# rongzhao-zhang/EfficientQ

Measured on AMD Instinct MI355X. Metric: ptq_calibration_throughput, higher is better.
Workload: dtype i8xi8->i32 (exact) for the Gram systems and per-iteration loss convs of the layers with quantised input, f32/f64 elsewhere

## Files before the change

### efficientq_amd/csrc/solve.hip

```cpp
#include <cstdlib>
#include <vector>
#include "common.h"

namespace effq {

typedef float f32x16 __attribute__((ext_vector_type(16)));
typedef double f64x4 __attribute__((ext_vector_type(4)));
typedef float f32x4 __attribute__((ext_vector_type(4)));

static inline int round_up(int v, int m) { return (v + m - 1) / m * m; }

constexpr int NBK = 64;
constexpr int LDA_S = 66;
constexpr int LDB_S = 80;

__global__ __launch_bounds__(256) void k_build_a64(const float* __restrict__ A0, int n, int npad, int has_bias,
                                                   double rho, double eta, double* __restrict__ A64) {
  const size_t tot = (size_t)npad * npad;
  const size_t stride = (size_t)gridDim.x * blockDim.x;
  for (size_t e = (size_t)blockIdx.x * blockDim.x + threadIdx.x; e < tot; e += stride) {
    const int i = (int)(e / npad), j = (int)(e % npad);
    double v = 0.0;
    if (i < n && j < n) {
      v = (double)A0[(size_t)i * n + j];
// ... 516 lines not shown
  constexpr int CPW = NBK / 16;
  auto invert64 = [&](int off) {
    double reg[CPW];
#pragma unroll
    for (int j = 0; j < CPW; ++j) reg[j] = M[(off + lane) * PF_LD + off + wid * CPW + j];
    gj_invert_regs<CPW>(reg, fcol, lane, wid);
#pragma unroll
    for (int j = 0; j < CPW; ++j) M[(off + lane) * PF_LD + off + wid * CPW + j] = reg[j];
    lds_barrier();
  };
  auto zero = []() {
    f64x4 z;
#pragma unroll
    for (int r = 0; r < 4; ++r) z[r] = 0.0;
    return z;
  };
  auto tile_store = [&](int rb, int cb, f64x4 v, double sgn) {
#pragma unroll
    for (int r = 0; r < 4; ++r) M[(rb + tr * 16 + lk + 4 * r) * PF_LD + cb + tc * 16 + lr] = sgn * v[r];
  };
  auto tile_load = [&](int rb, int cb) {
    f64x4 v;
#pragma unroll
    for (int r = 0; r < 4; ++r) v[r] = M[(rb + tr * 16 + lk + 4 * r) * PF_LD + cb + tc * 16 + lr];
    return v;
  };
  invert64(0);
  if (mk == 2) {
    f64x4 z = mm16(zero(), M + (NBK + tr * 16) * PF_LD, PF_LD, 1, M + tc * 16, PF_LD, 1, NBK, lr, lk);
    lds_barrier();
    tile_store(NBK, 0, z, 1.0);
    lds_barrier();
    f64x4 sacc = tile_load(NBK, NBK);
#pragma unroll
    for (int r = 0; r < 4; ++r) sacc[r] = -sacc[r];
    sacc = mm16(sacc, M + (NBK + tr * 16) * PF_LD, PF_LD, 1, M + NBK + tc * 16, PF_LD, 1, NBK, lr, lk);
    tile_store(NBK, NBK, sacc, -1.0);
    lds_barrier();
    invert64(NBK);
    f64x4 w = mm16(zero(), M + (NBK + tr * 16) * PF_LD + NBK, PF_LD, 1, M + NBK * PF_LD + tc * 16, PF_LD, 1, NBK, lr, lk);
    tile_store(0, NBK, w, 1.0);
    lds_barrier();
    f64x4 d = tile_load(0, 0);
    d = mm16(d, M + NBK * PF_LD + tr * 16, 1, PF_LD, M + NBK + tc * 16, PF_LD, 1, NBK, lr, lk);
    tile_store(0, 0, d, 1.0);
    lds_barrier();
  }
  const int nd = mk * NBK;
  for (int e = tid; e < nd * nd; e += 1024) {
    const int i = e / nd, j = e % nd;
    double v;
    if (i < NBK && j >= NBK)
      v = -M[(j - NBK) * PF_LD + NBK + i];
    else if (i >= NBK && j < NBK)
      v = -M[(i - NBK) * PF_LD + NBK + j];
    else
      v = M[i * PF_LD + j];
    Dw[e] = v;
  }
}

__global__ __launch_bounds__(256) void k_mirror_blocks(double* __restrict__ D, int nd) {
  const size_t tot = (size_t)nd * nd;
  for (size_t e = (size_t)blockIdx.x * blockDim.x + threadIdx.x; e < tot; e += (size_t)gridDim.x * blockDim.x) {
    const int i = (int)(e / nd), j = (int)(e % nd);
    if ((i / NBK) > (j / NBK)) D[e] = D[(size_t)j * nd + i];
  }
}

__global__ __launch_bounds__(256) void k_build_b(const float* __restrict__ B0, const float* __restrict__ W0,
                                                 const float* __restrict__ b0, const float* __restrict__ G,
                                                 const float* __restrict__ dual, int c2, int n, int has_bias,
                                                 float rho, float eta, float* __restrict__ Bm, int ldb, int c2p,
                                                 const float* __restrict__ wprev, float shift) {
  const size_t tot = (size_t)c2p * ldb;
  const size_t stride = (size_t)gridDim.x * blockDim.x;
  const int nw = n - has_bias;
  for (size_t e = (size_t)blockIdx.x * blockDim.x + threadIdx.x; e < tot; e += stride) {
    const int r = (int)(e / ldb), k = (int)(e % ldb);
    float v = 0.0f;
    if (r < c2 && k < n) {
      if (k < nw) {
        const size_t wi = (size_t)r * nw + k;
        v = B0[(size_t)r * n + k] + eta * W0[wi];
        v = v + rho * (G[wi] - dual[wi]);
        if (wprev != nullptr) v = v + shift * wprev[wi];
      } else {
        v = B0[(size_t)r * n + k] + eta * b0[r];
      }
    }
    Bm[e] = v;
  }
}

__global__ __launch_bounds__(256) void k_build_b4(const float* __restrict__ B0, const float* __restrict__ W0,
                                                  const float* __restrict__ b0, const float* __restrict__ G,
                                                  const float* __restrict__ dual, int c2, int n, int has_bias,
                                                  float rho, float eta, float* __restrict__ Bm, int ldb,
                                                  const float* __restrict__ wprev, float shift) {
  __builtin_amdgcn_s_setprio(2);

  const int r = blockIdx.y;
  const int nw = n - has_bias;
  float* out = Bm + (size_t)r * ldb;
  for (int k = (blockIdx.x * blockDim.x + threadIdx.x) * 4; k < ldb; k += gridDim.x * blockDim.x * 4) {
    float4 v = make_float4(0.f, 0.f, 0.f, 0.f);
    if (r < c2 && k < nw) {
      const size_t wi = (size_t)r * nw + k;
      const float* bp = B0 + (size_t)r * n + k;
      const float4 w0 = *reinterpret_cast<const float4*>(W0 + wi), g = *reinterpret_cast<const float4*>(G + wi),
                   du = *reinterpret_cast<const float4*>(dual + wi);
      v.x = bp[0] + eta * w0.x;
      v.y = bp[1] + eta * w0.y;
      v.z = bp[2] + eta * w0.z;
      v.w = bp[3] + eta * w0.w;
      v.x = v.x + rho * (g.x - du.x);
      v.y = v.y + rho * (g.y - du.y);
      v.z = v.z + rho * (g.z - du.z);
      v.w = v.w + rho * (g.w - du.w);
      if (wprev != nullptr) {
        const float4 wp = *reinterpret_cast<const float4*>(wprev + wi);
        v.x = v.x + shift * wp.x;
        v.y = v.y + shift * wp.y;
        v.z = v.z + shift * wp.z;
        v.w = v.w + shift * wp.w;
      }
    } else if (r < c2 && k == nw && has_bias) {
      v.x = B0[(size_t)r * n + k] + eta * b0[r];
    }
    *reinterpret_cast<float4*>(out + k) = v;
  }
}

__global__ __launch_bounds__(256) void k_prox_reduce4(const float* __restrict__ part, int ldp, int nsplit, int c2, int n,
                                                      int has_bias, float* __restrict__ wstar, float* __restrict__ bstar) {
  __builtin_amdgcn_s_setprio(2);

  const int r = blockIdx.y;
  const int nw = n - has_bias;
  const size_t tot = (size_t)c2 * ldp;
  const float* row = part + (size_t)r * ldp;
  for (int k = (blockIdx.x * blockDim.x + threadIdx.x) * 4; k < ldp; k += gridDim.x * blockDim.x * 4) {
    if (k >= n) continue;
    float4 v = *reinterpret_cast<const float4*>(row + k);
    for (int z = 1; z < nsplit; ++z) {
      const float4 t = *reinterpret_cast<const float4*>(row + (size_t)z * tot + k);
      v.x += t.x;
      v.y += t.y;
      v.z += t.z;
      v.w += t.w;
    }
    if (k < nw)
      *reinterpret_cast<float4*>(wstar + (size_t)r * nw + k) = v;
    else
      bstar[r] = v.x;
  }
}

constexpr int PBK = 32, PLD = PBK + 4;

template <int MT, int WM, int WN, int NTN>
__global__ __launch_bounds__(256) void k_prox_gemm(const float* __restrict__ Bm, int ldb, const float* __restrict__ Ainv,
                                                   int lda, int n, int c2, int has_bias, float* __restrict__ wstar,
                                                   float* __restrict__ bstar, float* __restrict__ part, int ldp) {
  __builtin_amdgcn_s_setprio(2);

  constexpr int BM = 32 * MT * WM, BN = 32 * WN * NTN;
  constexpr int NA = BM * 8 / 256, NB = BN * 8 / 256;
  static_assert(WM * WN == 4 && NA >= 1 && NB >= 1, "4 waves");
  __shared__ __attribute__((aligned(16))) float As[BM * PLD];
  __shared__ __attribute__((aligned(16))) float Bs[BN * PLD];
  const int tid = threadIdx.x, lane = tid & 63, wid = tid >> 6;
  const int li = lane & 31, lh = lane >> 5;
  const int wm = wid / WN, wn = wid % WN;
  const int row0 = blockIdx.y * BM, col0 = blockIdx.x * BN;

  f32x16 acc[MT][NTN];
#pragma unroll
  for (int m = 0; m < MT; ++m)
#pragma unroll
    for (int t = 0; t < NTN; ++t)
#pragma unroll
      for (int r = 0; r < 16; ++r) acc[m][t][r] = 0.0f;

  f32x4 ra[NA], rb[NB];
  const float* pa[NA];
  const float* pb[NB];
#pragma unroll
  for (int q = 0; q < NA; ++q) {
    const int u = tid + q * 256, r = u >> 3, c4 = u & 7;
    pa[q] = Bm + (size_t)(row0 + r) * ldb + c4 * 4;
  }
#pragma unroll
  for (int q = 0; q < NB; ++q) {
    const int u = tid + q * 256, r = u >> 3, c4 = u & 7;
    pb[q] = Ainv + (size_t)min(col0 + r, n - 1) * lda + c4 * 4;
  }
#define EFFQ_PROX_FETCH(k0)                                                         \
  {                                                                                 \
    _Pragma("unroll") for (int q = 0; q < NA; ++q)                                  \
        ra[q] = *reinterpret_cast<const f32x4*>(pa[q] + (k0));                      \
    _Pragma("unroll") for (int q = 0; q < NB; ++q)                                  \
        rb[q] = *reinterpret_cast<const f32x4*>(pb[q] + (k0));                      \
  }
  const int nkt = ldb / PBK;
  const int kt0 = (int)(((long long)nkt * blockIdx.z) / gridDim.z);
  const int nk = (int)(((long long)nkt * (blockIdx.z + 1)) / gridDim.z);
  EFFQ_PROX_FETCH(kt0 * PBK)
  for (int kt = kt0; kt < nk; ++kt) {
    lds_barrier();
#pragma unroll
    for (int q = 0; q < NA; ++q) {
      const int u = tid + q * 256;
      *reinterpret_cast<f32x4*>(&As[(u >> 3) * PLD + (u & 7) * 4]) = ra[q];
    }
#pragma unroll
    for (int q = 0; q < NB; ++q) {
      const int u = tid + q * 256;
      *reinterpret_cast<f32x4*>(&Bs[(u >> 3) * PLD + (u & 7) * 4]) = rb[q];
    }
    lds_barrier();
    EFFQ_PROX_FETCH(min(kt + 1, nk - 1) * PBK)
    __builtin_amdgcn_sched_barrier(0);
#pragma unroll
    for (int q = 0; q < 4; ++q) {
      f32x4 a[MT], b[NTN];
#pragma unroll
      for (int m = 0; m < MT; ++m)
        a[m] = *reinterpret_cast<const f32x4*>(&As[((wm * MT + m) * 32 + li) * PLD + q * 8 + 4 * lh]);
#pragma unroll
      for (int t = 0; t < NTN; ++t)
        b[t] = *reinterpret_cast<const f32x4*>(&Bs[((wn * NTN + t) * 32 + li) * PLD + q * 8 + 4 * lh]);
#pragma unroll
      for (int m = 0; m < MT; ++m)
#pragma unroll
        for (int t = 0; t < NTN; ++t)
#pragma unroll
          for (int e = 0; e < 4; ++e)
            acc[m][t] = __builtin_amdgcn_mfma_f32_32x32x2f32(a[m][e], b[t][e], acc[m][t], 0, 0, 0);
    }
  }
#undef EFFQ_PROX_FETCH
  const int nw = n - has_bias;
  if (gridDim.z > 1) {
    float* P = part + (size_t)blockIdx.z * c2 * ldp;
#pragma unroll
    for (int m = 0; m < MT; ++m)
#pragma unroll
      for (int t = 0; t < NTN; ++t) {
        const int col = col0 + (wn * NTN + t) * 32 + li;
#pragma unroll
        for (int r = 0; r < 16; ++r) {
          const int row = row0 + (wm * MT + m) * 32 + (r & 3) + 8 * (r >> 2) + 4 * lh;
          if (row < c2 && col < n) P[(size_t)row * ldp + col] = acc[m][t][r];
        }
      }
    return;
  }
#pragma unroll
  for (int m = 0; m < MT; ++m)
#pragma unroll
    for (int t = 0; t < NTN; ++t) {
      const int col = col0 + (wn * NTN + t) * 32 + li;
#pragma unroll
      for (int r = 0; r < 16; ++r) {
        const int row = row0 + (wm * MT + m) * 32 + (r & 3) + 8 * (r >> 2) + 4 * lh;
        if (row < c2 && col < n) {
          if (col < nw)
            wstar[(size_t)row * nw + col] = acc[m][t][r];
          else
            bstar[row] = acc[m][t][r];
        }
      }
    }
}


typedef __bf16 bf16x8 __attribute__((ext_vector_type(8)));
typedef __bf16 bf16x4 __attribute__((ext_vector_type(4)));
constexpr int B3_K = 16;
constexpr int B3_LD = B3_K + 8;

__device__ __forceinline__ void split3(const f32x4 v, bf16x4& p0, bf16x4& p1, bf16x4& p2) {
#pragma unroll
  for (int e = 0; e < 4; ++e) {
    const __bf16 b0 = (__bf16)v[e];
    const float r1 = v[e] - (float)b0;
    const __bf16 b1 = (__bf16)r1;
    const float r2 = r1 - (float)b1;
    p0[e] = b0;
    p1[e] = b1;
    p2[e] = (__bf16)r2;
  }
}

template <int BM, int BN, int WM, int WN>
__global__ __launch_bounds__(512) void k_prox_gemm_b3(const float* __restrict__ Bm, int ldb, const float* __restrict__ Ainv,
                                                      int lda, int n, int c2, int has_bias, float* __restrict__ wstar,
                                                      float* __restrict__ bstar, float* __restrict__ part, int ldp) {
  __builtin_amdgcn_s_setprio(2);
  constexpr int MT = BM / WM / 32, NT = BN / WN / 32;
  constexpr int NA = BM * 4 / 512, NB = BN * 4 / 512;
  constexpr int STAGE = 3 * (BM + BN) * B3_LD;
  static_assert(WM * WN == 8 && MT >= 1 && NT >= 1 && NA >= 1 && NB >= 1, "8 waves");
  extern __shared__ __attribute__((aligned(16))) unsigned char b3_lds[];
  __bf16* lds = reinterpret_cast<__bf16*>(b3_lds);
  const int tid = threadIdx.x, lane = tid & 63, wid = tid >> 6;
  const int li = lane & 31, lh = lane >> 5;
  const int wm = wid / WN, wn = wid % WN;
  const int row0 = blockIdx.y * BM, col0 = blockIdx.x * BN;

  f32x16 acc[MT][NT];
#pragma unroll
  for (int m = 0; m < MT; ++m)
#pragma unroll
    for (int t = 0; t < NT; ++t)
#pragma unroll
      for (int r = 0; r < 16; ++r) acc[m][t][r] = 0.0f;

  f32x4 ra[NA], rb[NB];
  const float* pa[NA];
  const float* pb[NB];
#pragma unroll
  for (int q = 0; q < NA; ++q) {
    const int u = tid + q * 512, r = u >> 2, c4 = u & 3;
    pa[q] = Bm + (size_t)(row0 + r) * ldb + c4 * 4;
  }
#pragma unroll
  for (int q = 0; q < NB; ++q) {
    const int u = tid + q * 512, r = u >> 2, c4 = u & 3;
    pb[q] = Ainv + (size_t)min(col0 + r, n - 1) * lda + c4 * 4;
  }
#define EFFQ_B3_FETCH(k0)                                                           \
  {                                                                                 \
    _Pragma("unroll") for (int q = 0; q < NA; ++q)                                  \
        ra[q] = *reinterpret_cast<const f32x4*>(pa[q] + (k0));                      \
    _Pragma("unroll") for (int q = 0; q < NB; ++q)                                  \
        rb[q] = *reinterpret_cast<const f32x4*>(pb[q] + (k0));                      \
  }
#define EFFQ_B3_STORE(stage)                                                                        \
  {                                                                                                 \
    __bf16* As_ = lds + (stage) * STAGE;                                                            \
    __bf16* Bs_ = As_ + 3 * BM * B3_LD;                                                             \
    _Pragma("unroll") for (int q = 0; q < NA; ++q) {                                                \
      const int u = tid + q * 512, off = (u >> 2) * B3_LD + (u & 3) * 4;                            \
      bf16x4 p0, p1, p2;                                                                            \
      split3(ra[q], p0, p1, p2);                                                                    \
      *reinterpret_cast<bf16x4*>(&As_[off]) = p0;                                                   \
      *reinterpret_cast<bf16x4*>(&As_[BM * B3_LD + off]) = p1;                                      \
      *reinterpret_cast<bf16x4*>(&As_[2 * BM * B3_LD + off]) = p2;                                  \
    }                                                                                               \
    _Pragma("unroll") for (int q = 0; q < NB; ++q) {                                                \
      const int u = tid + q * 512, off = (u >> 2) * B3_LD + (u & 3) * 4;                            \
      bf16x4 p0, p1, p2;                                                                            \
      split3(rb[q], p0, p1, p2);                                                                    \
      *reinterpret_cast<bf16x4*>(&Bs_[off]) = p0;                                                   \
      *reinterpret_cast<bf16x4*>(&Bs_[BN * B3_LD + off]) = p1;                                      \
      *reinterpret_cast<bf16x4*>(&Bs_[2 * BN * B3_LD + off]) = p2;                                  \
    }                                                                                               \
  }
  const int nkt = ldb / B3_K;
  const int kt0 = (int)(((long long)nkt * blockIdx.z) / gridDim.z);
  const int nk = (int)(((long long)nkt * (blockIdx.z + 1)) / gridDim.z);
  EFFQ_B3_FETCH(kt0 * B3_K)
  EFFQ_B3_STORE(0)
  EFFQ_B3_FETCH(min(kt0 + 1, nk - 1) * B3_K)
  lds_barrier();
  for (int kt = kt0; kt < nk; ++kt) {
    const int st = (kt - kt0) & 1;
    if (kt + 1 < nk) EFFQ_B3_STORE(st ^ 1)
    EFFQ_B3_FETCH(min(kt + 2, nk - 1) * B3_K)
    const __bf16* As = lds + st * STAGE;
    const __bf16* Bs = As + 3 * BM * B3_LD;
    bf16x8 a[MT][3], b[NT][3];
#pragma unroll
    for (int m = 0; m < MT; ++m)
#pragma unroll
      for (int p = 0; p < 3; ++p)
        a[m][p] = *reinterpret_cast<const bf16x8*>(&As[p * BM * B3_LD + ((wm * MT + m) * 32 + li) * B3_LD + 8 * lh]);
#pragma unroll
    for (int t = 0; t < NT; ++t)
#pragma unroll
      for (int p = 0; p < 3; ++p)
        b[t][p] = *reinterpret_cast<const bf16x8*>(&Bs[p * BN * B3_LD + ((wn * NT + t) * 32 + li) * B3_LD + 8 * lh]);
#pragma unroll
    for (int m = 0; m < MT; ++m)
#pragma unroll
      for (int t = 0; t < NT; ++t) {
        acc[m][t] = __builtin_amdgcn_mfma_f32_32x32x16_bf16(a[m][0], b[t][2], acc[m][t], 0, 0, 0);
        acc[m][t] = __builtin_amdgcn_mfma_f32_32x32x16_bf16(a[m][1], b[t][1], acc[m][t], 0, 0, 0);
        acc[m][t] = __builtin_amdgcn_mfma_f32_32x32x16_bf16(a[m][2], b[t][0], acc[m][t], 0, 0, 0);
        acc[m][t] = __builtin_amdgcn_mfma_f32_32x32x16_bf16(a[m][0], b[t][1], acc[m][t], 0, 0, 0);
        acc[m][t] = __builtin_amdgcn_mfma_f32_32x32x16_bf16(a[m][1], b[t][0], acc[m][t], 0, 0, 0);
        acc[m][t] = __builtin_amdgcn_mfma_f32_32x32x16_bf16(a[m][0], b[t][0], acc[m][t], 0, 0, 0);
      }
    lds_barrier();
  }
#undef EFFQ_B3_FETCH
#undef EFFQ_B3_STORE
  const int nw = n - has_bias;
  float* P = (gridDim.z > 1) ? part + (size_t)blockIdx.z * c2 * ldp : nullptr;
#pragma unroll
  for (int m = 0; m < MT; ++m)
#pragma unroll
    for (int t = 0; t < NT; ++t) {
      const int col = col0 + (wn * NT + t) * 32 + li;
#pragma unroll
      for (int r = 0; r < 16; ++r) {
        const int row = row0 + (wm * MT + m) * 32 + (r & 3) + 8 * (r >> 2) + 4 * lh;
        if (row < c2 && col < n) {
          if (P != nullptr)
            P[(size_t)row * ldp + col] = acc[m][t][r];
          else if (col < nw)
            wstar[(size_t)row * nw + col] = acc[m][t][r];
          else
            bstar[row] = acc[m][t][r];
        }
      }
    }
}

__global__ __launch_bounds__(256) void k_prox_reduce(const float* __restrict__ part, int ldp, int nsplit, int c2, int n,
                                                     int has_bias, float* __restrict__ wstar, float* __restrict__ bstar) {
  const size_t tot = (size_t)c2 * ldp, stride = (size_t)gridDim.x * blockDim.x;
  const int nw = n - has_bias;
  for (size_t e = (size_t)blockIdx.x * blockDim.x + threadIdx.x; e < tot; e += stride) {
    const int row = (int)(e / ldp), col = (int)(e % ldp);
    if (col >= n) continue;
    float v = part[e];
    for (int z = 1; z < nsplit; ++z) v += part[(size_t)z * tot + e];
    if (col < nw)
      wstar[(size_t)row * nw + col] = v;
    else
      bstar[row] = v;
  }
}

struct ProxPlan { int variant, gx, gy, nsplit, c2p, ldb; };
static ProxPlan prox_plan(int c2, int n) {
  ProxPlan p;
  p.c2p = (c2 > 128) ? round_up(c2, 256) : (c2 > 64) ? 128 : round_up(c2, 32);
  p.ldb = round_up(n, 32);
  if (p.c2p >= 128 && n >= 1024) {
    p.variant = 5; p.gx = (n + 255) / 256; p.gy = p.c2p / 256;
    if (p.c2p == 128) { p.variant = 7; p.gx = (n + 127) / 128; p.gy = 1; }
    const int tiles5 = p.gx * p.gy, nkt5 = p.ldb / B3_K;
    int s5 = (256 + tiles5 / 2) / tiles5;
    if (s5 > nkt5 / 16) s5 = nkt5 / 16;
    if (s5 < 1) s5 = 1;
    p.nsplit = s5;
    return p;
  }
  if (p.c2p >= 256) { p.variant = 0; p.gx = (n + 63) / 64; p.gy = p.c2p / 256; }
  else if (p.c2p == 128) { p.variant = 1; p.gx = (n + 63) / 64; p.gy = 1; }
  else if (p.c2p == 64) { p.variant = 2; p.gx = (n + 63) / 64; p.gy = 1; }
  else { p.variant = 3; p.gx = (n + 127) / 128; p.gy = 1; }
  const int tiles = p.gx * p.gy, nkt = p.ldb / PBK;
  int s = (440 + tiles - 1) / tiles;
  if (s > nkt / 6) s = nkt / 6;
  if (s > 16) s = 16;
  if (s < 1) s = 1;
  if (p.variant == 0) {
    const int smax = s > 1 ? 16 : 1;
    double best = -1.0;
    for (int c = 1; c <= smax && c <= nkt / 6; ++c) {
      const int wgs = tiles * c, rounds = (wgs + 767) / 768;
      const double score = (double)wgs / (768.0 * rounds) - 0.01 * c;
      if (score > best) { best = score; s = c; }
    }
  }
  p.nsplit = s;
  return p;
}

}

using namespace effq;

extern "C" {

static size_t gj64_aux_doubles(size_t npad) { return 2 * (size_t)NBK * npad + 2 * NBK * NBK; }

constexpr int GJ_WIDE_MIN_BLOCKS = 100;

size_t effq_spd_inverse_ws_bytes(int n) {
  if (n <= 0) return 0;
  const size_t npad = (size_t)round_up(n, NBK);
  size_t d = npad * npad + gj64_aux_doubles(npad);
  if ((int)(npad / NBK) >= GJ_WIDE_MIN_BLOCKS) {
    const size_t ldx = (size_t)round_up((int)npad, BG_T);
    d = npad * npad + 2 * (size_t)WK * ldx + (size_t)WK * WK + gj64_aux_doubles(WK);
  }
  return d * sizeof(double) + 256;
}

int effq_ainv_ld(int n) { return n > 0 ? round_up(n, 32) : 0; }

static int gj64_sweep(double* A64, int npad, double* aux, hipStream_t st) {
  const int nblk = npad / NBK;
  double* XT = aux;
  double* NZ = XT + (size_t)NBK * npad;
  double* Dinv = NZ + (size_t)NBK * npad;
  const size_t lds = (size_t)(NBK * LDA_S + NBK * LDB_S) * sizeof(double);
  for (int k = 0; k < nblk; ++k) {
    const int kb = k * NBK;
    double* Dk = Dinv + (size_t)(k & 1) * NBK * NBK;
    double* Dn = Dinv + (size_t)((k + 1) & 1) * NBK * NBK;
    if (k == 0) hipLaunchKernelGGL(k_gj_diag, dim3(1), dim3(GJD_T), 0, st, A64, npad, kb, Dk);
    hipLaunchKernelGGL(k_gj_panel, dim3(nblk), dim3(256), lds, st, A64, npad, kb, Dk, NZ, XT);
    if (nblk > 1)
      hipLaunchKernelGGL(k_gj_trail_sym, dim3((nblk + GJ_CT - 1) / GJ_CT, nblk + 1), dim3(256), 0, st, A64, npad, kb, NZ,
                         XT, Dn);
    EFFQ_LAUNCH_CHECK();
  }
  return EFFQ_OK;
}

struct GjWideCtx {
  int dev;
  hipStream_t caller, helper;
  hipEvent_t e1, e2;
};
static thread_local std::vector<GjWideCtx> g_gj_ctx;

static int gj_wide_ctx(hipStream_t caller, GjWideCtx** out) {
  int dev = 0;
  EFFQ_HIP(hipGetDevice(&dev));
  for (GjWideCtx& c : g_gj_ctx)
    if (c.dev == dev && c.caller == caller) {
      *out = &c;
      return EFFQ_OK;
    }
  GjWideCtx c;
  c.dev = dev;
  c.caller = caller;
  int prio = 0;
  if (hipStreamGetPriority(caller, &prio) != hipSuccess) prio = 0;
  EFFQ_HIP(hipStreamCreateWithPriority(&c.helper, hipStreamNonBlocking, prio));
  EFFQ_HIP(hipEventCreateWithFlags(&c.e1, hipEventDisableTiming));
  EFFQ_HIP(hipEventCreateWithFlags(&c.e2, hipEventDisableTiming));
  g_gj_ctx.push_back(c);
  *out = &g_gj_ctx.back();
  return EFFQ_OK;
}

static int gj_wide_sweep(double* A64, int npad, double* aux, hipStream_t st) {
  const int nblk = npad / NBK;
  const int WB = (nblk >= 100) ? effq::WB : 2;
  const size_t ldx = (size_t)round_up(npad, BG_T);
  double* NZT = aux;
  double* XTW = NZT + (size_t)WK * ldx;
  double* Dw = XTW + (size_t)WK * ldx;
  double* aux64 = Dw + (size_t)WK * WK;
  const int nK = (nblk + WB - 1) / WB, nm = (nblk + 1) / 2;
  GjWideCtx* ctx = nullptr;
  if (nK > 1) {
    const int rc = gj_wide_ctx(st, &ctx);
    if (rc != EFFQ_OK) return rc;
  }
  hipStream_t s2 = ctx ? ctx->helper : st;
  const size_t lds = (size_t)(NBK * LDA_S + NBK * LDB_S) * sizeof(double);
  const size_t pf_lds = (size_t)(2 * NBK * PF_LD + 2 * (NBK + 1)) * sizeof(double);
  auto pivot_block = [&](int k0, int mk, int kdim, hipStream_t s) -> int {
    GjBig g;
    memset(&g, 0, sizeof(g));
    g.Cin = A64; g.ldin = (size_t)npad;
    g.Cout = Dw; g.ldout = (size_t)mk * NBK; g.orow = k0 * NBK; g.ocol = k0 * NBK;
    g.NZT = NZT; g.XTW = XTW; g.ldx = ldx; g.kdim = kdim; g.nblk = nblk;
    g.i0m = k0 / 2; g.j0m = k0 / 2;
    g.skip_lo = g.skip_hi = -1; g.la_lo = g.la_hi = -1;
    if (WB == 2) {
      hipLaunchKernelGGL(k_gj_pivot_fused, dim3(1), dim3(1024), pf_lds, s, A64, npad, k0, mk, NZT, XTW, ldx, kdim, Dw);
      EFFQ_LAUNCH_CHECK();
      return EFFQ_OK;
    }
    const int span = (mk + 1) / 2;
    hipLaunchKernelGGL(k_gj_big, dim3(span, span), dim3(256), 0, s, g);
    EFFQ_LAUNCH_CHECK();
    const int rc = gj64_sweep(Dw, mk * NBK, aux64, s);
    if (rc != EFFQ_OK) return rc;
    hipLaunchKernelGGL(k_mirror_blocks, dim3(64), dim3(256), 0, s, Dw, mk * NBK);
    EFFQ_LAUNCH_CHECK();
    return EFFQ_OK;
  };
  {
    const int rc = pivot_block(0, nblk < WB ? nblk : WB, 0, st);
    if (rc != EFFQ_OK) return rc;
  }
  for (int K = 0; K < nK; ++K) {
    const int kb0 = K * WB, m = (nblk - kb0 < WB) ? nblk - kb0 : WB;
    const int kn0 = kb0 + WB, mn = (K + 1 < nK) ? ((nblk - kn0 < WB) ? nblk - kn0 : WB) : 0;
    hipLaunchKernelGGL(k_gj_panel_w, dim3(nblk, m), dim3(256), lds, st, A64, npad, kb0, m, Dw, NZT, XTW, ldx);
    EFFQ_LAUNCH_CHECK();
    if (ctx) {
      EFFQ_HIP(hipEventRecord(ctx->e1, st));
      EFFQ_HIP(hipStreamWaitEvent(s2, ctx->e1, 0));
    }
    hipLaunchKernelGGL(k_gj_wback_w, dim3(nblk, m), dim3(256), 0, s2, A64, npad, kb0, m, Dw, NZT, ldx);
    EFFQ_LAUNCH_CHECK();
    if (mn > 0) {
      const int rc = pivot_block(kn0, mn, m * NBK, s2);
      if (rc != EFFQ_OK) return rc;
    }
    if (nblk > m) {
      GjBig g;
      memset(&g, 0, sizeof(g));
      g.Cin = A64; g.ldin = (size_t)npad;
      g.Cout = A64; g.ldout = (size_t)npad; g.orow = 0; g.ocol = 0;
      g.NZT = NZT; g.XTW = XTW; g.ldx = ldx; g.kdim = m * NBK; g.nblk = nblk;
      g.i0m = 0; g.j0m = 0;
      g.skip_lo = kb0; g.skip_hi = kb0 + m;
      g.la_lo = mn > 0 ? kn0 : -1; g.la_hi = mn > 0 ? kn0 + mn : -1;
      hipLaunchKernelGGL(k_gj_big, dim3(nm, nm), dim3(256), 0, st, g);
      EFFQ_LAUNCH_CHECK();
    }
    if (ctx) {
      EFFQ_HIP(hipEventRecord(ctx->e2, s2));
      EFFQ_HIP(hipStreamWaitEvent(st, ctx->e2, 0));
    }
  }
  return EFFQ_OK;
}

int effq_spd_inverse_prepare(void* stream) {
  GjWideCtx* ctx = nullptr;
  return gj_wide_ctx(as_stream(stream), &ctx);
}

int effq_spd_inverse(const float* A0, int n, int has_bias, double rho, double eta, float* Ainv, void* ws,
                     size_t ws_bytes, void* stream) {
  EFFQ_CHECK_ARG(A0 && Ainv && ws && n > 0);
  EFFQ_CHECK_ARG(eta > 0.0 && rho >= 0.0);
  if (ws_bytes < effq_spd_inverse_ws_bytes(n)) {
    set_error("spd_inverse: workspace %zu < required %zu", ws_bytes, effq_spd_inverse_ws_bytes(n));
    return EFFQ_ERR_WORKSPACE;
  }
  const int npad = round_up(n, NBK);
  double* A64 = reinterpret_cast<double*>(ws);
  double* aux = A64 + (size_t)npad * npad;
  hipStream_t st = as_stream(stream);
  {
    size_t nb = ((size_t)npad * npad + 255) / 256;
    if (nb > 8192) nb = 8192;
    hipLaunchKernelGGL(k_build_a64, dim3((unsigned)nb), dim3(256), 0, st, A0, n, npad, has_bias, rho, eta, A64);
    EFFQ_LAUNCH_CHECK();
  }
  const size_t lds = (size_t)(NBK * LDA_S + NBK * LDB_S) * sizeof(double);
  static bool attr_set = false;
  if (!attr_set) {
    EFFQ_HIP(hipFuncSetAttribute(reinterpret_cast<const void*>(k_gj_panel), hipFuncAttributeMaxDynamicSharedMemorySize, (int)lds));
    EFFQ_HIP(hipFuncSetAttribute(reinterpret_cast<const void*>(k_gj_panel_w), hipFuncAttributeMaxDynamicSharedMemorySize, (int)lds));
    EFFQ_HIP(hipFuncSetAttribute(reinterpret_cast<const void*>(k_gj_pivot_fused), hipFuncAttributeMaxDynamicSharedMemorySize,
                                 (int)((2 * NBK * PF_LD + 2 * (NBK + 1)) * sizeof(double))));
    attr_set = true;
  }
  const int rc = (npad / NBK >= GJ_WIDE_MIN_BLOCKS) ? gj_wide_sweep(A64, npad, aux, st) : gj64_sweep(A64, npad, aux, st);
  if (rc != EFFQ_OK) return rc;
  {
    const int lda = effq_ainv_ld(n);
    size_t nb = ((size_t)n * lda + 255) / 256;
    if (nb > 8192) nb = 8192;
    hipLaunchKernelGGL(k_a64_to_f32, dim3((unsigned)nb), dim3(256), 0, st, A64, n, npad, Ainv, lda);
    EFFQ_LAUNCH_CHECK();
  }
  return EFFQ_OK;
}

size_t effq_prox_ws_bytes(int c2, int n) {
  if (c2 <= 0 || n <= 0) return 0;
  const ProxPlan p = prox_plan(c2, n);
  return ((size_t)p.c2p + (p.nsplit > 1 ? (size_t)p.nsplit * c2 : 0)) * p.ldb * sizeof(float) + 256;
}

static int prox_solve_impl(const float* B0, const float* Ainv, const float* W0, const float* b0, const float* G,
                           const float* dual, int c2, int n, int has_bias, double rho, double eta, double shift,
                           int nterms, float* wstar, float* bstar, void* ws, size_t ws_bytes, void* stream,
                           bool prebuilt = false, const float** part_out = nullptr, int* nsplit_out = nullptr,
                           int* ldp_out = nullptr) {
  EFFQ_CHECK_ARG(B0 && Ainv && W0 && G && dual && wstar && ws && c2 > 0 && n > 0 && nterms >= 1);
  EFFQ_CHECK_ARG(!has_bias || (b0 != nullptr && bstar != nullptr));
  if (ws_bytes < effq_prox_ws_bytes(c2, n)) {
    set_error("prox_solve: workspace %zu < required %zu", ws_bytes, effq_prox_ws_bytes(c2, n));
    return EFFQ_ERR_WORKSPACE;
  }
  const ProxPlan pl = prox_plan(c2, n);
  const int c2p = pl.c2p, ldb = pl.ldb;
  const int lda = effq_ainv_ld(n);
  float* Bm = reinterpret_cast<float*>(ws);
  float* part = Bm + (size_t)c2p * ldb;
  hipStream_t st = as_stream(stream);
  for (int term = 0; term < nterms; ++term) {
    if (!(prebuilt && term == 0)) {
      const int nw = n - (has_bias ? 1 : 0);
      if ((nw % 4) == 0) {
        const unsigned bx = (unsigned)((ldb / 4 + 255) / 256);
        hipLaunchKernelGGL(k_build_b4, dim3(bx, (unsigned)c2p), dim3(256), 0, st, B0, W0, b0, G, dual, c2, n,
                           has_bias ? 1 : 0, (float)rho, (float)eta, Bm, ldb, (term > 0) ? wstar : nullptr, (float)shift);
      } else {
        size_t nb = ((size_t)c2p * ldb + 255) / 256;
        if (nb > 4096) nb = 4096;
// ... 101 lines not shown
```

Baseline: 24.91.

## Interleave split-bf16 LDS stores and prefetch with MFMA groups in prox GEMM

Restructures the k-loop of the 3-way split-bf16 prox GEMM. The single store-then-compute step becomes six MFMA groups, with each group followed by one piece of the next tile's split/LDS store and global prefetch. sched_group_barrier hints make the compiler interleave MFMA, VALU and memory instructions. It also permutes the rows each thread writes to LDS and precomputes the store offsets, likely to reduce bank conflicts. In exchange it adds register pressure, relies on exact compiler scheduling hints, and now does a redundant store on the last iteration.

Result: no change. 25.02, median of 6 (+0.5%).

```diff
diff --git a/efficientq_amd/csrc/solve.hip b/efficientq_amd/csrc/solve.hip
--- a/efficientq_amd/csrc/solve.hip
+++ b/efficientq_amd/csrc/solve.hip
@@ -842,7 +842,8 @@
   constexpr int MT = BM / WM / 32, NT = BN / WN / 32;
   constexpr int NA = BM * 4 / 512, NB = BN * 4 / 512;
   constexpr int STAGE = 3 * (BM + BN) * B3_LD;
-  static_assert(WM * WN == 8 && MT >= 1 && NT >= 1 && NA >= 1 && NB >= 1, "8 waves");
+  static_assert(WM * WN == 8 && MT >= 1 && NT >= 1 && NA >= 1 && NB >= 1 && NA + NB <= 4, "8 waves");
+#define PIECE_GROUP(q) ((q) * 6 / (NA + NB))
   extern __shared__ __attribute__((aligned(16))) unsigned char b3_lds[];
   __bf16* lds = reinterpret_cast<__bf16*>(b3_lds);
   const int tid = threadIdx.x, lane = tid & 63, wid = tid >> 6;
@@ -861,81 +862,119 @@
   f32x4 ra[NA], rb[NB];
   const float* pa[NA];
   const float* pb[NB];
+  int sa[NA], sb[NB];
 #pragma unroll
   for (int q = 0; q < NA; ++q) {
-    const int u = tid + q * 512, r = u >> 2, c4 = u & 3;
+    const int u = tid + q * 512, r = ((u >> 5) << 3) | (((u >> 2) & 3) << 1) | ((u >> 4) & 1), c4 = u & 3;
     pa[q] = Bm + (size_t)(row0 + r) * ldb + c4 * 4;
+    sa[q] = r * B3_LD + c4 * 4;
   }
 #pragma unroll
   for (int q = 0; q < NB; ++q) {
-    const int u = tid + q * 512, r = u >> 2, c4 = u & 3;
+    const int u = tid + q * 512, r = ((u >> 5) << 3) | (((u >> 2) & 3) << 1) | ((u >> 4) & 1), c4 = u & 3;
     pb[q] = Ainv + (size_t)min(col0 + r, n - 1) * lda + c4 * 4;
-  }
-#define EFFQ_B3_FETCH(k0)                                                           \
+    sb[q] = r * B3_LD + c4 * 4;
+  }
+#define EFFQ_B3_FETCH(RA, RB, k0)                                                   \
   {                                                                                 \
     _Pragma("unroll") for (int q = 0; q < NA; ++q)                                  \
-        ra[q] = *reinterpret_cast<const f32x4*>(pa[q] + (k0));                      \
+        RA[q] = *reinterpret_cast<const f32x4*>(pa[q] + (k0));                      \
     _Pragma("unroll") for (int q = 0; q < NB; ++q)                                  \
-        rb[q] = *reinterpret_cast<const f32x4*>(pb[q] + (k0));                      \
-  }
-#define EFFQ_B3_STORE(stage)                                                                        \
+        RB[q] = *reinterpret_cast<const f32x4*>(pb[q] + (k0));                      \
+  }
+#define EFFQ_B3_STORE(RA, RB, stage)                                                                \
   {                                                                                                 \
     __bf16* As_ = lds + (stage) * STAGE;                                                            \
     __bf16* Bs_ = As_ + 3 * BM * B3_LD;                                                             \
     _Pragma("unroll") for (int q = 0; q < NA; ++q) {                                                \
-      const int u = tid + q * 512, off = (u >> 2) * B3_LD + (u & 3) * 4;                            \
       bf16x4 p0, p1, p2;                                                                            \
-      split3(ra[q], p0, p1, p2);                                                                    \
-      *reinterpret_cast<bf16x4*>(&As_[off]) = p0;                                                   \
-      *reinterpret_cast<bf16x4*>(&As_[BM * B3_LD + off]) = p1;                                      \
-      *reinterpret_cast<bf16x4*>(&As_[2 * BM * B3_LD + off]) = p2;                                  \
+      split3(RA[q], p0, p1, p2);                                                                    \
+      *reinterpret_cast<bf16x4*>(&As_[sa[q]]) = p0;                                                 \
+      *reinterpret_cast<bf16x4*>(&As_[BM * B3_LD + sa[q]]) = p1;                                    \
+      *reinterpret_cast<bf16x4*>(&As_[2 * BM * B3_LD + sa[q]]) = p2;                                \
     }                                                                                               \
     _Pragma("unroll") for (int q = 0; q < NB; ++q) {                                                \
-      const int u = tid + q * 512, off = (u >> 2) * B3_LD + (u & 3) * 4;                            \
       bf16x4 p0, p1, p2;                                                                            \
-      split3(rb[q], p0, p1, p2);                                                                    \
-      *reinterpret_cast<bf16x4*>(&Bs_[off]) = p0;                                                   \
-      *reinterpret_cast<bf16x4*>(&Bs_[BN * B3_LD + off]) = p1;                                      \
-      *reinterpret_cast<bf16x4*>(&Bs_[2 * BN * B3_LD + off]) = p2;                                  \
+      split3(RB[q], p0, p1, p2);                                                                    \
+      *reinterpret_cast<bf16x4*>(&Bs_[sb[q]]) = p0;                                                 \
+      *reinterpret_cast<bf16x4*>(&Bs_[BN * B3_LD + sb[q]]) = p1;                                    \
+      *reinterpret_cast<bf16x4*>(&Bs_[2 * BN * B3_LD + sb[q]]) = p2;                                \
     }                                                                                               \
+  }
+#define EFFQ_B3_PIECE(q, ostage)                                                                                        \
+  {                                                                                                                     \
+    __bf16* As_ = lds + (ostage) * STAGE;                                                                               \
+    __bf16* Bs_ = As_ + 3 * BM * B3_LD;                                                                                 \
+    bf16x4 p0, p1, p2;                                                                                                  \
+    if ((q) < NA) {                                                                                                     \
+      constexpr int qa = (q) < NA ? (q) : 0;                                                                            \
+      split3(ra[qa], p0, p1, p2);                                                                                       \
+      *reinterpret_cast<bf16x4*>(&As_[sa[qa]]) = p0;                                                                    \
+      *reinterpret_cast<bf16x4*>(&As_[BM * B3_LD + sa[qa]]) = p1;                                                       \
+      *reinterpret_cast<bf16x4*>(&As_[2 * BM * B3_LD + sa[qa]]) = p2;                                                   \
+      ra[qa] = *reinterpret_cast<const f32x4*>(pa[qa] + k2);                                                            \
+    } else {                                                                                                            \
+      constexpr int qb = (q) >= NA ? (q) - NA : 0;                                                                      \
+      split3(rb[qb], p0, p1, p2);                                                                                       \
+      *reinterpret_cast<bf16x4*>(&Bs_[sb[qb]]) = p0;                                                                    \
+      *reinterpret_cast<bf16x4*>(&Bs_[BN * B3_LD + sb[qb]]) = p1;                                                       \
+      *reinterpret_cast<bf16x4*>(&Bs_[2 * BN * B3_LD + sb[qb]]) = p2;                                                   \
+      rb[qb] = *reinterpret_cast<const f32x4*>(pb[qb] + k2);                                                            \
+    }                                                                                                                   \
+  }
+#define EFFQ_B3_GROUP(j, stage)                                                                                         \
+  {                                                                                                                     \
+    constexpr int pa_ = (j) < 3 ? (j) : (j) < 5 ? (j) - 3 : 0, pb_ = (j) < 3 ? 2 - (j) : (j) < 5 ? 4 - (j) : 0;         \
+    _Pragma("unroll") for (int m = 0; m < MT; ++m)                                                                      \
+      _Pragma("unroll") for (int t = 0; t < NT; ++t)                                                                    \
+        acc[m][t] = __builtin_amdgcn_mfma_f32_32x32x16_bf16(a[m][pa_], b[t][pb_], acc[m][t], 0, 0, 0);                  \
+    if (PIECE_GROUP(0) == (j)) EFFQ_B3_PIECE(0, (stage) ^ 1)                                                            \
+    if (NA + NB > 1 && PIECE_GROUP(1) == (j)) EFFQ_B3_PIECE(1, (stage) ^ 1)                                             \
+    if (NA + NB > 2 && PIECE_GROUP(2) == (j)) EFFQ_B3_PIECE(2, (stage) ^ 1)                                             \
+    if (NA + NB > 3 && PIECE_GROUP(3) == (j)) EFFQ_B3_PIECE(3, (stage) ^ 1)                                             \
+          \
+    _Pragma("unroll") for (int i = 0; i < MT * NT; ++i) {                                                               \
+      __builtin_amdgcn_sched_group_barrier(0x002, 4, 0);                                                               \
+      __builtin_amdgcn_sched_group_barrier(0x008, 1, 0);                                                               \
+      if (i & 1) __builtin_amdgcn_sched_group_barrier(0x200, 1, 0);                                                    \
+    }                                                                                                                   \
+    __builtin_amdgcn_sched_barrier(0);                                                                                  \
+  }
+#define EFFQ_B3_STEP(stage)                                                                                             \
+  {                                                                                                                     \
+    const __bf16* As = lds + (stage) * STAGE;                                                                           \
+    const __bf16* Bs = As + 3 * BM * B3_LD;                                                                             \
+    const int k2 = min(kt + 2, nk - 1) * B3_K;                                                                          \
+    bf16x8 a[MT][3], b[NT][3];                                                                                          \
+                                                           \
+    _Pragma("unroll") for (int j = 0; j < 3; ++j) {                                                                     \
+      _Pragma("unroll") for (int m = 0; m < MT; ++m)                                                                    \
+        a[m][j] = *reinterpret_cast<const bf16x8*>(&As[j * BM * B3_LD + ((wm * MT + m) * 32 + li) * B3_LD + 8 * lh]);  \
+      _Pragma("unroll") for (int t = 0; t < NT; ++t)                                                                    \
+        b[t][2 - j] =                                                                                                   \
+            *reinterpret_cast<const bf16x8*>(&Bs[(2 - j) * BN * B3_LD + ((wn * NT + t) * 32 + li) * B3_LD + 8 * lh]); \
+    }                                                                                                                   \
+    __builtin_amdgcn_sched_barrier(0);                                                                                  \
+    EFFQ_B3_GROUP(0, stage)                                                                                             \
+    EFFQ_B3_GROUP(1, stage)                                                                                             \
+    EFFQ_B3_GROUP(2, stage)                                                                                             \
+    EFFQ_B3_GROUP(3, stage)                                                                                             \
+    EFFQ_B3_GROUP(4, stage)                                                                                             \
+    EFFQ_B3_GROUP(5, stage)                                                                                             \
+    lds_barrier();                          \
   }
   const int nkt = ldb / B3_K;
   const int kt0 = (int)(((long long)nkt * blockIdx.z) / gridDim.z);
   const int nk = (int)(((long long)nkt * (blockIdx.z + 1)) / gridDim.z);
-  EFFQ_B3_FETCH(kt0 * B3_K)
-  EFFQ_B3_STORE(0)
-  EFFQ_B3_FETCH(min(kt0 + 1, nk - 1) * B3_K)
+  EFFQ_B3_FETCH(ra, rb, kt0 * B3_K)
+  EFFQ_B3_STORE(ra, rb, 0)
+  EFFQ_B3_FETCH(ra, rb, min(kt0 + 1, nk - 1) * B3_K)
   lds_barrier();
-  for (int kt = kt0; kt < nk; ++kt) {
-    const int st = (kt - kt0) & 1;
-    if (kt + 1 < nk) EFFQ_B3_STORE(st ^ 1)
-    EFFQ_B3_FETCH(min(kt + 2, nk - 1) * B3_K)
-    const __bf16* As = lds + st * STAGE;
-    const __bf16* Bs = As + 3 * BM * B3_LD;
-    bf16x8 a[MT][3], b[NT][3];
-#pragma unroll
-    for (int m = 0; m < MT; ++m)
-#pragma unroll
-      for (int p = 0; p < 3; ++p)
-        a[m][p] = *reinterpret_cast<const bf16x8*>(&As[p * BM * B3_LD + ((wm * MT + m) * 32 + li) * B3_LD + 8 * lh]);
-#pragma unroll
-    for (int t = 0; t < NT; ++t)
-#pragma unroll
-      for (int p = 0; p < 3; ++p)
-        b[t][p] = *reinterpret_cast<const bf16x8*>(&Bs[p * BN * B3_LD + ((wn * NT + t) * 32 + li) * B3_LD + 8 * lh]);
-#pragma unroll
-    for (int m = 0; m < MT; ++m)
-#pragma unroll
-      for (int t = 0; t < NT; ++t) {
-        acc[m][t] = __builtin_amdgcn_mfma_f32_32x32x16_bf16(a[m][0], b[t][2], acc[m][t], 0, 0, 0);
-        acc[m][t] = __builtin_amdgcn_mfma_f32_32x32x16_bf16(a[m][1], b[t][1], acc[m][t], 0, 0, 0);
-        acc[m][t] = __builtin_amdgcn_mfma_f32_32x32x16_bf16(a[m][2], b[t][0], acc[m][t], 0, 0, 0);
-        acc[m][t] = __builtin_amdgcn_mfma_f32_32x32x16_bf16(a[m][0], b[t][1], acc[m][t], 0, 0, 0);
-        acc[m][t] = __builtin_amdgcn_mfma_f32_32x32x16_bf16(a[m][1], b[t][0], acc[m][t], 0, 0, 0);
-        acc[m][t] = __builtin_amdgcn_mfma_f32_32x32x16_bf16(a[m][0], b[t][0], acc[m][t], 0, 0, 0);
-      }
-    lds_barrier();
-  }
+  for (int kt = kt0; kt < nk; ++kt) EFFQ_B3_STEP((kt - kt0) & 1)
+#undef EFFQ_B3_STEP
+#undef EFFQ_B3_GROUP
+#undef EFFQ_B3_PIECE
+#undef PIECE_GROUP
 #undef EFFQ_B3_FETCH
 #undef EFFQ_B3_STORE
   const int nw = n - has_bias;
```
